# stjude-rust-labs/ngs

Measured on AMD Instinct MI355X. Metric: BAM records/sec (whole node), all qc facets, 150 bp reads, higher is better.
Workload: dtype u8/u32 integer (u64 accumulators)

## Files before the change

ngs_amd/csrc/context.cpp:

```cpp
#include <dlfcn.h>
#include <hip/hip_runtime_api.h>

#include <algorithm>
#include <atomic>
#include <cstdarg>
#include <cstdlib>
#include <cstdio>
#include <cstring>
#include <string>
#include <thread>
#include <vector>

#include "../../include/ngsq.h"
#include "../../include/ngsq_shared.h"
#include "context.h"
#include "mem_pool.h"

using namespace ngsq;

namespace ngsq {
void free_exchange_scratch(void *p);
}

static thread_local std::string g_err;
// ... 239 lines not shown
        c->n_td = round_up(c->n_cov_hist + n_bins + NGSQ_VAF_BINS, 8);
        CTX_TRY(hipMalloc((void **)&c->d_td, c->n_td * 8));
        CTX_TRY(hipMemsetAsync(c->d_td, 0, c->n_td * 8, c->stream));
        c->d_cov_hist = c->d_td;
        c->d_bin_totals = c->d_td + c->n_cov_hist;
        c->d_vaf = c->d_td + c->n_cov_hist + n_bins;
        CTX_TRY(hipMalloc((void **)&c->d_touched, 16));
        CTX_TRY(hipMemcpyAsync(c->d_touched, c->h_touched, 16, hipMemcpyHostToDevice, c->stream));
        st.touched = c->d_touched;
    }
    c->stream_cov = c->cfg.sorted_input && nd;
    if (c->stream_cov) {
        const uint64_t nr4 = round_up(nr ? nr : 1, 4);
        CTX_TRY(hipMalloc((void **)&c->d_stream_u32, (7 * nr4 + 4) * 4));
        CTX_TRY(hipMalloc((void **)&c->d_last_key, 8));
        CTX_TRY(hipMalloc((void **)&c->d_chunk_flags, round_up(c->n_chunks ? c->n_chunks : 1, 16)));
        st.end_acc = c->d_stream_u32;
        st.batch_span = c->d_stream_u32 + 7 * nr4;
        CovStreamArgs &sa = c->csa;
        sa.prev_end = c->d_stream_u32 + nr4;
        sa.plan_a = c->d_stream_u32 + 2 * nr4;
        sa.plan_z = c->d_stream_u32 + 3 * nr4;
        sa.plan_h = c->d_stream_u32 + 4 * nr4;
        sa.plan_t = c->d_stream_u32 + 5 * nr4;
        sa.guard_until = c->d_stream_u32 + 6 * nr4;
        sa.last_key = c->d_last_key;
        sa.chunk_flags = c->d_chunk_flags;
        sa.hist = c->d_cov_hist;
        sa.bin_totals = c->d_bin_totals;
        sa.bin_off = c->d_bin_off;
        sa.bin_size = c->cfg.bin_size;
        sa.cov_cap = c->cfg.cov_cap;
        sa.head_guard = c->cfg.cov_head_guard;
        CTX_TRY(hipMemsetAsync(c->d_stream_u32, 0, (7 * nr4 + 4) * 4, c->stream));
        CTX_TRY(hipMemsetAsync(sa.plan_a, 0xFF, nr4 * 4, c->stream));
        CTX_TRY(hipMemsetAsync(c->d_last_key, 0, 8, c->stream));
        CTX_TRY(hipMemsetAsync(c->d_chunk_flags, 0, c->n_chunks ? c->n_chunks : 1, c->stream));
    }
    if (ne) {
        CTX_TRY(hipMalloc((void **)&st.edits, ne * 4 + 64));
        CTX_TRY(hipMemsetAsync(st.edits, 0, ne * 4 + 64, c->stream));
        uint8_t *bases = nullptr;
        CTX_TRY(hipMalloc((void **)&bases, 2 * nbases + 256));
        CTX_TRY(hipMemsetAsync(bases, 0, 2 * nbases + 256, c->stream));
        st.ref_bases = bases;
        st.ref_bases_odd = bases + nbases;
        c->d_ref_bases = bases;
        uint8_t *codes = nullptr;
        unsigned long long *d_bad = nullptr, h_bad = 0;
        CTX_TRY(hipMalloc((void **)&codes, (deferred ? 0 : max_len) + 64));
        CTX_TRY(hipMalloc((void **)&d_bad, 8));
        CTX_TRY(hipMemsetAsync(d_bad, 0, 8, c->stream));
        uint64_t n_carry = 0;
        c->edits_carry_off.assign(nr, 0);
        std::vector<uint32_t> have(2 * (size_t)nr, 0);
        bool lens_differ = false;
        for (uint32_t r = 0; r < nr; r++) {
            if (bases_off[r] == NO_DEPTH) continue;
            const uint64_t L = c->ref_len[r];
            const uint64_t have_r = cfg->ref_bases_len && !deferred ? std::min<uint64_t>(cfg->ref_bases_len[r], L) : L;
            have[nr + r] = (uint32_t)have_r;
            have[r] = cfg->ref_bases_len && !deferred ? cfg->ref_bases_len[r] : (uint32_t)L;
            lens_differ = lens_differ || have[r] != L;
            if (!deferred && have_r) {
                CTX_TRY(hipMemcpyAsync(codes, cfg->ref_bases[r], have_r, hipMemcpyHostToDevice, c->stream));
                CTX_TRY(launch_pack_reference(c->li, codes, have_r, bases + bases_off[r], bases + nbases + bases_off[r], L / 2 + 1, d_bad, c->stream));
// ... 4 lines not shown
        }
        if (lens_differ) {
            CTX_TRY(hipMalloc((void **)&c->d_edits_len, have.size() * 4));
            CTX_TRY(hipMemcpy(c->d_edits_len, have.data(), have.size() * 4, hipMemcpyHostToDevice));
            st.ref_edits_len = c->d_edits_len;
            st.ref_fast_len = c->d_edits_len + nr;
        }
        CTX_TRY(hipStreamSynchronize(c->stream));
        CTX_TRY(hipMemcpy(&h_bad, d_bad, 8, hipMemcpyDeviceToHost));
        (void)hipFree(codes);
        (void)hipFree(d_bad);
        if (h_bad) {
            ngsq_destroy(c);
            return fail(nullptr, NGSQ_ERR_INVALID_ARGUMENT, "ngsq_config.ref_bases: every byte must be a 4-bit BAM base code (0..15)");
        }
        CTX_TRY(hipMalloc((void **)&c->d_edits_carry, (n_carry + 4) * 4));
        c->edits_conv_lo.assign(nr, 0);
        c->edits_conv_hi.assign(nr, 0);
    }
    c->h_vaf.assign(NGSQ_VAF_BINS, 0);
    for (int k = 0; k < K_COUNT; k++) c->timing[k] = {KERNEL_NAMES[k], 0, 0.0, 0};
    CTX_TRY(hipStreamSynchronize(c->stream));
#undef CTX_TRY
    *out = c;
    return NGSQ_OK;
}

void ngsq_destroy(ngsq_ctx *c) {
    if (!c) return;
    (void)hipSetDevice(c->device);
    ngsq::reference_abandon(c);
    (void)ngsq::pool_trim();
    if (c->stream) (void)hipStreamSynchronize(c->stream);
    (void)hipFree(c->d_ft_idx);
    (void)hipFree(c->d_ft_starts);
    (void)hipFree(c->d_ft_stops);
    (void)hipFree(c->d_ft_primary);
    for (const ngsq_ctx::DeferredFeatures &d : c->ft_deferred) (void)hipFree(d.buf);
    for (auto &p : c->pending) {
        (void)hipEventDestroy(p.a);
        (void)hipEventDestroy(p.b);
    }
    for (auto &ev : c->event_pool) (void)hipEventDestroy(ev);
    for (int k = 0; k < 2; k++) {
        if (c->stage[k].buf) (void)hipFree(c->stage[k].buf);
        if (c->stage[k].done) (void)hipEventDestroy(c->stage[k].done);
    }
    if (c->copy_done) (void)hipEventDestroy(c->copy_done);
    (void)hipFree(c->st.counters);
    (void)hipFree(c->st.depth);
    (void)hipFree(c->st.edits);
    (void)hipFree(c->d_ref_bases);
    (void)hipFree(c->d_edits_len);
    (void)hipFree(c->d_bad_off);
    (void)hipFree(c->d_bad_pos);
    (void)hipFree(c->d_edits_carry);
    (void)hipFree(c->d_edits_td);
    (void)hipFree(c->d_edits_defer);
    (void)hipFree(c->d_ref_len);
    (void)hipFree(c->d_depth_off);
    (void)hipFree(c->d_edits_off);
    (void)hipFree(c->d_bases_off);
    (void)hipFree(c->d_first_chunk);
    (void)hipFree(c->d_bin_off);
    (void)hipFree(c->d_td);
    (void)hipFree(c->d_touched);
// ... 124 lines not shown
        off += round_up(n ? n : 1, 256);
        return p;
    }
};

struct ColumnSizes {
    uint64_t seq_bytes, qual_bytes, cigar_ops;
};

static int column_sizes(ngsq_ctx *c, const ngsq_batch *b, ColumnSizes *cs) {
    const uint64_t n = b->n_records;
    const bool host = b->location == NGSQ_MEM_HOST;
    cs->seq_bytes = b->seq_bytes;
    cs->qual_bytes = b->qual_bytes;
    cs->cigar_ops = b->cigar_ops;
    if (!b->seq) cs->seq_bytes = 0;
    else if (!b->seq_off) cs->seq_bytes = n * b->seq_stride;
    else if (host) cs->seq_bytes = b->seq_off[n];
    if (!b->qual) cs->qual_bytes = 0;
    else if (!b->qual_off) cs->qual_bytes = n * b->qual_stride;
    else if (host) cs->qual_bytes = b->qual_off[n];
    if (!b->cigar) cs->cigar_ops = 0;
    else if (!b->cigar_off) cs->cigar_ops = n * b->cigar_stride;
    else if (host) cs->cigar_ops = b->cigar_off[n];
    (void)c;
    return NGSQ_OK;
}

static int launch_all(ngsq_ctx *c, const DeviceBatch &db, const ColumnSizes &cs, uint32_t pass_mask) {
    const uint32_t facets = c->cfg.facets;
    const uint64_t n = db.n;
    const uint32_t rec_f = (pass_mask & NGSQ_PASS_RECORD) ? (facets & NGSQ_FACETS_RECORD_BASED) : 0;
    const uint32_t seq_f = (pass_mask & NGSQ_PASS_SEQUENCE) ? (facets & NGSQ_FACETS_SEQUENCE_BASED) : 0;
    if ((rec_f & (NGSQ_FACET_GENERAL | NGSQ_FACET_TEMPLATE_LENGTH)) || (seq_f & NGSQ_FACET_COVERAGE)) {
        const bool walk = (rec_f & NGSQ_FACET_GENERAL) || (seq_f & NGSQ_FACET_COVERAGE);
        const bool cov = (seq_f & NGSQ_FACET_COVERAGE) != 0;
        if (cov && c->stream_cov) {
            const uint64_t need = round_up(n, 1024) + 1024;
            if (c->cov_end_cap < need) {
                HIP_TRY(c, hipStreamSynchronize(c->stream));
                (void)hipFree(c->d_cov_end);
                c->d_cov_end = nullptr;
                c->cov_end_cap = 0;
                HIP_TRY(c, hipMalloc((void **)&c->d_cov_end, need * 4));
                c->cov_end_cap = need;
                c->st.cov_end = c->d_cov_end;
            }
            uint32_t *const spans = c->d_stream_u32 + 7 * round_up(c->st.n_refs ? c->st.n_refs : 1, 4);
            c->st.batch_span = spans + (c->span_turn & 1);
            c->csa.span_next = spans + ((c->span_turn & 1) ^ 1);
            c->span_turn += 1;
        }
        {
            Bracket br(c, K_FIELDS, n * 25 + (walk ? cs.cigar_ops * 4 : 0));
            HIP_TRY(c, launch_fields(c->li, c->st, db, rec_f, cov ? (c->stream_cov ? 2 : 1) : 0, c->stream));
        }
        if (cov && c->stream_cov) {
            Bracket br(c, K_COV_STREAM, n * 8);
            HIP_TRY(c, launch_cov_stream(c->li, c->st, db, c->csa, c->stream));
        }
    }
    const bool gc_in_edits = (rec_f & NGSQ_FACET_GC_CONTENT) && (seq_f & NGSQ_FACET_EDITS) && edits_can_take_gc(c->st, db);
    if ((rec_f & NGSQ_FACET_GC_CONTENT) && !gc_in_edits) {
        Bracket br(c, K_GC, n * 6 + cs.seq_bytes);
        HIP_TRY(c, launch_gc(c->li, c->st, db, cs.seq_bytes, c->stream));
    }
    if (rec_f & NGSQ_FACET_QUALITY_SCORE) {
        Bracket br(c, K_QUAL, cs.qual_bytes);
        HIP_TRY(c, launch_qual(c->li, c->st, db, c->stream));
    }
    if (rec_f & NGSQ_FACET_FEATURES) {
        if (!c->have_features) {
            ngsq_ctx::DeferredFeatures d{nullptr, 0, n};
            const uint64_t n16 = round_up(n, 16);
            HIP_TRY(c, ngsq::pool_device_alloc((void **)&d.buf, n16 * 16 + 256, &d.bytes));
            c->ft_deferred.push_back(d);
            Bracket br(c, K_FEATURES, n * 12 + cs.cigar_ops * 4);
            HIP_TRY(c, launch_features_defer(c->li, db, reinterpret_cast<uint16_t *>(d.buf + n16 * 12), reinterpret_cast<int32_t *>(d.buf),
                                             reinterpret_cast<int32_t *>(d.buf + n16 * 4), reinterpret_cast<uint16_t *>(d.buf + n16 * 14),
                                             reinterpret_cast<uint32_t *>(d.buf + n16 * 8), c->stream));
        } else {
            Bracket br(c, K_FEATURES, n * 12 + cs.cigar_ops * 4);
            HIP_TRY(c, launch_features(c->li, c->st, db, c->ft, c->stream));
        }
    }
    if (seq_f & NGSQ_FACET_EDITS) {
        if (c->ref_deferred && !c->ref_ready) {
            if (!c->ref_loader) return fail(c, NGSQ_ERR_STATE, "ngsq_config.ref_bases_deferred is set but ngsq_reference_load was not called");
            const int rc = reference_join(c);
            if (rc != NGSQ_OK) return rc;
        }
        Bracket br(c, K_EDITS, n * 16 + cs.cigar_ops * 4 + cs.seq_bytes);
        const uint64_t words = (n + 63) / 64 + 16;
        if (c->edits_defer_cap < words) {
            HIP_TRY(c, hipStreamSynchronize(c->stream));
            (void)hipFree(c->d_edits_defer);
            c->d_edits_defer = nullptr;
            c->edits_defer_cap = 0;
// ... 740 lines not shown
```

ngs_amd/csrc/context.h:

```cpp
#pragma once

#include <hip/hip_runtime_api.h>

#include <string>
#include <vector>

#include "../../include/ngsq.h"
#include "kernels.h"

struct ngsq_ctx;

namespace ngsq {

enum KernelId { K_FIELDS = 0, K_GC, K_QUAL, K_EDITS, K_COV_SCAN, K_EDITS_VAF, K_H2D, K_FEATURES, K_COV_STREAM, K_INFLATE, K_INFLATE_CRC,
                K_REC_INDEX, K_REC_COLUMNS, K_COUNT };

struct PendingTime {
    int id;
    hipEvent_t a, b;
};

struct KernelTimer {
    ngsq_ctx *c;
    int id;
// ... 39 lines not shown
    uint32_t *d_edits_carry = nullptr;
    uint8_t *d_edits_td = nullptr;
    size_t edits_td_cap = 0;
    std::vector<uint8_t> h_edits_td;
    unsigned long long *d_edits_defer = nullptr;
    uint64_t edits_defer_cap = 0;
    std::vector<uint64_t> edits_carry_off, edits_conv_lo, edits_conv_hi;
    uint32_t *d_first_chunk = nullptr;
    uint64_t *d_bin_off = nullptr;
    uint64_t n_diff = 0, n_chunks = 0;
    unsigned long long *d_td = nullptr;
    uint64_t n_td = 0;
    unsigned long long *d_touched = nullptr;
    unsigned long long h_touched[2] = {~0ull, 0};
    uint64_t scan_lo = 0, scan_hi = 0;
    uint32_t scan_carry = 0;
    const uint32_t *scan_words = nullptr;
    uint64_t scan_front = 0;
    uint32_t vaf_part = 0, vaf_parts = 1;
    void *xchg_scratch = nullptr;
    bool scan_partial = false, torn_down = false;
    unsigned long long *d_cov_hist = nullptr, *d_bin_totals = nullptr, *d_vaf = nullptr;
    std::vector<unsigned long long> h_counters, h_cov_hist, h_bin_totals, h_vaf;
    bool finalized = false;
    bool edits_uploaded = false;
    unsigned long long *pin_results = nullptr, *pin_results_dev = nullptr;
    uint64_t pin_words = 0;
    bool stream_cov = false;
    uint32_t *d_cov_end = nullptr;
    uint64_t cov_end_cap = 0;
    uint32_t *d_stream_u32 = nullptr;
    unsigned long long *d_last_key = nullptr;
    uint32_t span_turn = 0;
    uint8_t *d_chunk_flags = nullptr;
    ngsq::CovStreamArgs csa{};
    ngsq::FeatureTables ft{};
    uint32_t *d_ft_idx = nullptr, *d_ft_starts = nullptr, *d_ft_stops = nullptr;
    uint8_t *d_ft_primary = nullptr;
    bool have_features = false;
    struct DeferredFeatures {
        uint8_t *buf;
        size_t bytes;
        uint64_t n;
    };
    std::vector<DeferredFeatures> ft_deferred;
    ngsq::Staging stage[2];
    int stage_next = 0;
    ngsq_kernel_time timing[ngsq::K_COUNT]{};
    std::vector<ngsq::PendingTime> pending;
    std::vector<hipEvent_t> event_pool;
    std::string err;
};
```

ngs_amd/csrc/cov_stream.hip:

```cpp
#include <hip/hip_runtime.h>

#include <type_traits>

#include "kernels.h"

namespace ngsq {

typedef unsigned long long u64;

constexpr uint32_t ST_THREADS = 256;
constexpr uint32_t ST_WAVES = ST_THREADS / 64;
constexpr uint32_t ST_W = 1024;
constexpr uint32_t ST_LIST = 232;
constexpr uint32_t ST_HOT_BINS = 64, ST_HOT_REP = 4, ST_HOT = ST_HOT_BINS * ST_HOT_REP;

__device__ __forceinline__ u64 st_key(int32_t rf, int32_t ps) {
    return rf < 0 ? 0xFFFFFFFF00000000ull : ((u64)(uint32_t)rf << 32) | (uint32_t)(ps + 1);
}
__device__ __forceinline__ bool st_valid(const DeviceState &st, int32_t rf, int32_t ps) {
    return rf >= 0 && (uint32_t)rf < st.n_refs && ps >= 0 && st.ref_depth_off[rf] != NO_DEPTH;
}

__global__ __launch_bounds__(256) void k_cov_plan_tiles(DeviceState st, DeviceBatch b, CovStreamArgs a) {
    NGSQ_FOREGROUND_WAVE();
// ... 3 lines not shown
        const u64 k0 = st_key(b.ref_id[0], b.pos[0]);
        if (k0 < *a.last_key) atomicAdd(&st.counters[C_COV_UNSORTED], 1ull);
        *a.last_key = st_key(b.ref_id[b.n - 1], b.pos[b.n - 1]);
    }
    const uint32_t lane = threadIdx.x & 63u;
    auto first_of = [&](int64_t u, int32_t &r, int32_t &p) {
        const bool ok = u >= 0 && (uint64_t)u < n_wt;
        r = ok ? b.ref_id[(uint64_t)u * CS_TILE] : -1;
        p = ok ? b.pos[(uint64_t)u * CS_TILE] : -1;
    };
    int32_t rf[4], ps[4];
    first_of((int64_t)t, rf[1], ps[1]);
    rf[0] = __shfl_up(rf[1], 1, 64), ps[0] = __shfl_up(ps[1], 1, 64);
    rf[2] = __shfl_down(rf[1], 1, 64), ps[2] = __shfl_down(ps[1], 1, 64);
    rf[3] = __shfl_down(rf[1], 2, 64), ps[3] = __shfl_down(ps[1], 2, 64);
    if (lane == 0) first_of((int64_t)t - 1, rf[0], ps[0]);
    if (lane == 63) first_of((int64_t)t + 1, rf[2], ps[2]);
    if (lane >= 62) first_of((int64_t)t + 2, rf[3], ps[3]);
    if (t >= n_wt) return;
    auto streamable = [&](int k) {
        return st_valid(st, rf[k], ps[k]) && rf[k + 1] == rf[k] && ps[k + 1] >= 0;
    };
    if (!streamable(1)) return;
    const bool prev_same = streamable(0) && rf[0] == rf[1];
    const bool next_same = streamable(2) && rf[2] == rf[1];
    if (!prev_same) atomicMin(&a.plan_a[rf[1]], (uint32_t)ps[1] + 1);
    if (!next_same) atomicMax(&a.plan_z[rf[1]], (uint32_t)ps[2] + 1);
}

__global__ __launch_bounds__(256) void k_cov_plan_refs(DeviceState st, CovStreamArgs a) {
    NGSQ_FOREGROUND_WAVE();
    const uint32_t r = blockIdx.x * blockDim.x + threadIdx.x;
    if (r == 0 && a.span_next) *a.span_next = 0;
    if (r >= st.n_refs) return;
    const uint32_t pa = a.plan_a[r], pz = a.plan_z[r], prev = a.prev_end[r];
    const uint32_t acc = st.end_acc[r];
    uint32_t guard = a.guard_until[r];
    if (a.head_guard && guard == 0 && (pa != CS_NONE || acc != 0)) {
        const uint64_t g = (uint64_t)(pa != CS_NONE ? pa : acc) + a.head_guard;
        guard = g > 0xFFFFFFFEull ? 0xFFFFFFFEu : (uint32_t)g;
        a.guard_until[r] = guard;
    }
    uint32_t H = CS_NONE, T = CS_NONE;
    if (pa != CS_NONE && pz > pa) {
        uint64_t base = pa > prev + 1 ? pa : (uint64_t)prev + 1;
        if (guard > base) base = guard;
        const uint64_t h = (base + COV_CHUNK - 1) / COV_CHUNK * COV_CHUNK;
        const uint64_t lim = pz < (uint64_t)st.ref_len[r] + 1 ? pz : (uint64_t)st.ref_len[r] + 1;
        const uint64_t tt = lim / COV_CHUNK * COV_CHUNK;
        if (h < tt) {
            H = (uint32_t)h;
            T = (uint32_t)tt;
        }
    }
    a.plan_h[r] = H;
    a.plan_t[r] = T;
    a.prev_end[r] = acc > prev ? acc : prev;
    a.plan_a[r] = CS_NONE;
    a.plan_z[r] = 0;
}

__device__ __forceinline__ uint32_t st_wave_scan(uint32_t v) {
    v += (uint32_t)__builtin_amdgcn_update_dpp(0, (int)v, 0x111, 0xF, 0xF, false);
    v += (uint32_t)__builtin_amdgcn_update_dpp(0, (int)v, 0x112, 0xF, 0xF, false);
    v += (uint32_t)__builtin_amdgcn_update_dpp(0, (int)v, 0x114, 0xF, 0xF, false);
    v += (uint32_t)__builtin_amdgcn_update_dpp(0, (int)v, 0x118, 0xF, 0xF, false);
    v += (uint32_t)__builtin_amdgcn_update_dpp(0, (int)v, 0x142, 0xA, 0xF, false);
    v += (uint32_t)__builtin_amdgcn_update_dpp(0, (int)v, 0x143, 0xC, 0xF, false);
    return v;
}
__device__ __forceinline__ uint32_t st_wave_max(uint32_t v) {
#pragma unroll
    for (int o = 32; o > 0; o >>= 1) v = max(v, (uint32_t)__shfl_xor(v, o, 64));
    return v;
}

__host__ __device__ inline uint32_t st_hist_words(uint32_t cov_cap) { return ((cov_cap + 2 + 1) / 2 + 3) & ~3u; }

constexpr uint32_t ST_PER_LANE = 8;
constexpr uint32_t ST_PASS = 64 * ST_PER_LANE;
static_assert(ST_W % ST_PASS == 0, "whole passes");

struct StTileIn {
    int4 p;
    uint4 c;
    int32_t rf_t, ps_t, rf_n, ps_n;
};

constexpr uint32_t ST_MIN_BLOCKS = 4;
__global__ __launch_bounds__(ST_THREADS, ST_MIN_BLOCKS) void k_cov_stream(DeviceState st, DeviceBatch b, CovStreamArgs a) {
    NGSQ_FOREGROUND_WAVE();
    extern __shared__ __attribute__((aligned(16))) uint32_t s_dyn[];
    const uint32_t nb = a.cov_cap + 2;
    const uint32_t tid = threadIdx.x, lane = tid & 63;
    const uint32_t wave = (uint32_t)__builtin_amdgcn_readfirstlane((int)(tid >> 6));
    const uint32_t hw = st_hist_words(a.cov_cap);
    uint32_t *const win = s_dyn + wave * (ST_W + hw + ST_HOT + ST_LIST);
    uint32_t *const hist = win + ST_W;
    uint32_t *const hot = hist + hw;
    uint32_t *const lst = hot + ST_HOT;
    for (uint32_t i = lane; i < ST_W + hw + ST_HOT + ST_LIST; i += 64) win[i] = 0;
    __builtin_amdgcn_fence(__ATOMIC_ACQ_REL, "wavefront");
    __builtin_amdgcn_wave_barrier();

    const uint64_t n_wt = (b.n + CS_TILE - 1) / CS_TILE;
    const uint64_t n_full = b.n / CS_TILE;
    const uint64_t n_units = (uint64_t)gridDim.x * ST_WAVES, unit = (uint64_t)blockIdx.x * ST_WAVES + wave;
    const uint64_t per = (n_wt + n_units - 1) / n_units;
    const uint64_t t_begin = per * unit < n_wt ? per * unit : n_wt;
    const uint64_t t_end = t_begin + per < n_wt ? t_begin + per : n_wt;
    const uint32_t maxspan = *st.batch_span;

    uint32_t hot_base = 0;
    int32_t hist_ref = -1;
    uint32_t since_flush = 0;
    u64 zero_run = 0;
    uint32_t lane_zero = 0;
    u64 *bins = a.bin_totals;
    u64 lane_bin = 0;
    uint32_t bin_q = 0, bin_p0 = 1, bin_p1 = 0;
    u64 t_lo = ~0ull, t_hi = 0;
    bool lst_valid = false;
    uint64_t lst_tile = 0;
    int32_t lst_ref = -1;
    uint32_t lst_lo = 0, lst_n = 0;
    int32_t plan_ref = -1;
    uint32_t pH = CS_NONE, pT = CS_NONE, pL = 0;
    uint64_t pOff = 0;

    auto flush_bin = [&]() {
        u64 v = lane_bin;
#pragma unroll
        for (int o = 32; o > 0; o >>= 1) v += __shfl_xor(v, o, 64);
        if (lane == 0 && v) atomicAdd(&bins[bin_q], v);
        lane_bin = 0;
    };
    auto flush_hot = [&]() {
        static_assert((ST_HOT_REP == 4 || ST_HOT_REP == 8) && ST_HOT_BINS <= 64, "one or two uint4 per lane");
        uint4 *const cell = reinterpret_cast<uint4 *>(hot) + (lane < ST_HOT_BINS ? lane : 0u) * (ST_HOT_REP / 4);
        uint32_t t = 0;
        if (lane < ST_HOT_BINS) {
#pragma unroll
            for (uint32_t q = 0; q < ST_HOT_REP / 4; q++) {
// ... 303 lines not shown
                    __builtin_amdgcn_wave_barrier();
                }
            }
        }

        if (from_list) {
            for (uint32_t c = 0; c < lst_n; c += 64) {
                const uint32_t ee = c + lane < lst_n ? lst[c + lane] : 0u;
                const u64 km = __ballot(ee > hi);
                if (ee > hi) lst[new_n + __builtin_amdgcn_mbcnt_hi((uint32_t)(km >> 32), __builtin_amdgcn_mbcnt_lo((uint32_t)km, 0))] = ee;
                new_n += (uint32_t)__popcll(km);
            }
        }
#pragma unroll
        for (uint32_t j = 0; j < 4; j++) {
            const u64 km = __ballot(e[j] > hi);
            const uint32_t kn = (uint32_t)__popcll(km);
            if (new_ok && new_n + kn <= ST_LIST) {
                if (e[j] > hi) lst[new_n + __builtin_amdgcn_mbcnt_hi((uint32_t)(km >> 32), __builtin_amdgcn_mbcnt_lo((uint32_t)km, 0))] = e[j];
                new_n += kn;
            } else {
                new_ok = false;
            }
        }
        lst_valid = new_ok;
        lst_n = new_n;
        lst_tile = t + 1;
        lst_ref = rf_t;
        lst_lo = hi;
        __builtin_amdgcn_fence(__ATOMIC_ACQ_REL, "wavefront");
        __builtin_amdgcn_wave_barrier();
    };

    uint64_t t = t_begin;
    const uint64_t t_full_end = t_end < n_full ? t_end : n_full;
    if (t < t_full_end) {
        StTileIn cur = load_full(t);
        while (t < t_full_end) {
            const uint64_t tn = t + 1;
            const StTileIn nxt = load_full(tn < n_full ? tn : t);
            process(cur, t);
            cur = nxt;
            t = tn;
        }
    }
    if (n_full < n_wt && t_begin <= n_full && n_full < t_end) {
        const uint64_t base = n_full * CS_TILE, r0 = base + (uint64_t)lane * 4;
        int32_t p[4];
        uint32_t c[4];
#pragma unroll
        for (uint32_t j = 0; j < 4; j++) {
            const bool ok = r0 + j < b.n;
            p[j] = ok ? b.pos[r0 + j] : -1;
            c[j] = ok ? st.cov_end[r0 + j] : 0u;
        }
        StTileIn in;
        in.p = make_int4(p[0], p[1], p[2], p[3]);
        in.c = make_uint4(c[0], c[1], c[2], c[3]);
        in.rf_t = in.rf_n = b.ref_id[base];
        in.ps_t = in.ps_n = b.pos[base];
        process(in, n_full);
    }
    flush_hist();
    flush_bin();
#pragma unroll
    for (int o = 32; o > 0; o >>= 1) {
        const u64 l2 = __shfl_xor(t_lo, o, 64), h2 = __shfl_xor(t_hi, o, 64);
        t_lo = l2 < t_lo ? l2 : t_lo;
        t_hi = h2 > t_hi ? h2 : t_hi;
    }
    if (lane == 0 && t_hi > 0) {
        atomicMin(&st.touched[0], t_lo);
        atomicMax(&st.touched[1], t_hi);
    }
}

hipError_t launch_cov_stream(const LaunchInfo &li, const DeviceState &st, const DeviceBatch &b, const CovStreamArgs &a,
                             hipStream_t s) {
    if (!b.n) return hipSuccess;
    const uint64_t n_wt = (b.n + CS_TILE - 1) / CS_TILE;
    hipLaunchKernelGGL(k_cov_plan_tiles, dim3((uint32_t)((n_wt + 255) / 256)), dim3(256), 0, s, st, b, a);
    hipLaunchKernelGGL(k_cov_plan_refs, dim3((st.n_refs + 255) / 256), dim3(256), 0, s, st, a);
    const size_t lds = (size_t)ST_WAVES * (ST_W + st_hist_words(a.cov_cap) + ST_HOT + ST_LIST) * sizeof(uint32_t);
    static bool attr = false;
    if (!attr) {
        hipError_t e = hipFuncSetAttribute(reinterpret_cast<const void *>(k_cov_stream),
                                           hipFuncAttributeMaxDynamicSharedMemorySize, 160 * 1024 - 64);
        if (e != hipSuccess) return e;
        attr = true;
    }
    uint64_t g = (n_wt + ST_WAVES - 1) / ST_WAVES;
    const uint64_t per_cu = (160 * 1024 - 1024) / lds;
    const uint64_t cap = (uint64_t)li.n_cu * (per_cu < 1 ? 1 : per_cu > 6 ? 6 : per_cu);
    if (g > cap) g = cap;
    hipLaunchKernelGGL(k_cov_stream, dim3((uint32_t)g), dim3(ST_THREADS), lds, s, st, b, a);
    return hipGetLastError();
}

}
```

ngs_amd/csrc/kernels.h:

```cpp
#pragma once

#include <hip/hip_runtime_api.h>
#include <stdint.h>

#include "../../include/ngsq.h"

#define NGSQ_FOREGROUND_WAVE() __builtin_amdgcn_s_setprio(3)

namespace ngsq {

enum : uint32_t {
    C_GENERAL = 0,
    C_CIGAR1 = 16,
    C_CIGAR2 = 25,
    C_TLEN_PROCESSED = 34,
    C_TLEN_IGNORED = 35,
    C_GC_GC = 36,
    C_GC_AT = 37,
    C_GC_OTHER = 38,
    C_GC_PROCESSED = 39,
    C_GC_IGN_FLAGS = 40,
    C_GC_IGN_SHORT = 41,
    C_COV_NONSENSICAL = 42,
    C_ERR = 43,
    E_MISSING_REF = 0,
    E_BAD_QUAL = 1,
    E_READ_TOO_LONG = 2,
    E_EDITS_BAD_REF = 3,
    E_EDITS_SHORT = 4,
    E_EDITS_NOT_CONSUMED = 5,
    E_EDITS_TOO_MANY = 6,
    E_BAD_CIGAR = 7,
    C_FEAT = 51,
    F_UTR5 = 0,
    F_UTR3 = 1,
    F_CDS = 2,
    F_INTERGENIC = 3,
    F_EXONIC = 4,
    F_INTRONIC = 5,
    F_PROCESSED = 6,
// ... 57 lines not shown
    const uint64_t *record_id;
    uint64_t qual_bytes;
};

#if defined(__HIPCC__)
__device__ __forceinline__ uint32_t batch_n_ops(const DeviceBatch &b, uint64_t i) {
    uint32_t n = b.n_cigar[i];
    if (n == 0xFFFFu && b.cigar_off) n = (uint32_t)(b.cigar_off[i + 1] - b.cigar_off[i]);
    return n;
}
#endif

struct LaunchInfo {
    int n_cu;
};

hipError_t launch_fields(const LaunchInfo &li, const DeviceState &st, const DeviceBatch &b,
                         uint32_t rec_facets, int coverage, hipStream_t s);

constexpr uint32_t CS_TILE = 256;
constexpr uint32_t CS_NONE = 0xFFFFFFFFu;
struct CovStreamArgs {
    uint32_t *plan_a, *plan_z;
    uint32_t *plan_h, *plan_t;
    uint32_t *prev_end;
    uint32_t *guard_until;
    unsigned long long *last_key;
    uint8_t *chunk_flags;
    unsigned long long *hist;
    unsigned long long *bin_totals;
    const uint64_t *bin_off;
    uint32_t bin_size, cov_cap, head_guard;
    uint32_t *span_next;
};
hipError_t launch_cov_stream(const LaunchInfo &li, const DeviceState &st, const DeviceBatch &b, const CovStreamArgs &a,
                             hipStream_t s);
hipError_t launch_gc(const LaunchInfo &li, const DeviceState &st, const DeviceBatch &b,
                     uint64_t seq_bytes, hipStream_t s);
hipError_t launch_qual(const LaunchInfo &li, const DeviceState &st, const DeviceBatch &b,
                       hipStream_t s);
bool qual_window_supported(const DeviceState &st, const DeviceBatch &b);
hipError_t launch_qual_window(const LaunchInfo &li, const DeviceState &st, const DeviceBatch &b, hipStream_t s);
struct FeatureTables {
    const uint32_t *idx;
    const uint32_t *starts;
    const uint32_t *stops;
    const uint8_t *primary;
    uint32_t n_refs;
    uint32_t role_name[5];
    unsigned long long *scratch;
};
constexpr uint32_t FT_SLOTS = 32;
hipError_t launch_features_defer(const LaunchInfo &li, const DeviceBatch &b, uint16_t *flag, int32_t *ref, int32_t *pos, uint16_t *ncig, uint32_t *cig,
                                 hipStream_t s);
hipError_t launch_features(const LaunchInfo &li, const DeviceState &st, const DeviceBatch &b, const FeatureTables &ft,
                           hipStream_t s);
bool qual_ragged_supported(const DeviceState &st, const DeviceBatch &b);
hipError_t launch_qual_ragged(const LaunchInfo &li, const DeviceState &st, const DeviceBatch &b, hipStream_t s);
bool edits_can_take_gc(const DeviceState &st, const DeviceBatch &b);
hipError_t launch_edits(const LaunchInfo &li, const DeviceState &st, const DeviceBatch &b, unsigned long long *defer_bits, bool with_gc,
                        hipStream_t s);

constexpr uint32_t COV_CHUNK = 4096;
constexpr uint32_t COV_SUPER = 256;
struct CovScanArgs {
    uint32_t *depth;
    uint64_t n_chunks;
    uint64_t c_begin, c_end;
    uint32_t carry_in;
    const uint32_t *carry_words;
    uint64_t carry_mask;
// ... 75 lines not shown
```

ngs_amd/csrc/kernels.hip:

```cpp
#include <hip/hip_runtime.h>

#include "../../include/ngsq_shared.h"
#include "kernels.h"

namespace ngsq {

typedef unsigned long long u64;

__device__ __forceinline__ uint32_t wave_sum(uint32_t v) {
#pragma unroll
    for (int o = 32; o > 0; o >>= 1) v += __shfl_down(v, o, 64);
    return v;
}
__device__ __forceinline__ u64 wave_sum64(u64 v) {
#pragma unroll
    for (int o = 32; o > 0; o >>= 1) v += __shfl_down(v, o, 64);
    return v;
}

template <int N>
__device__ __forceinline__ void block_flush(const uint32_t (&v)[N], u64 *s_acc, u64 *dst,
                                            const uint32_t (&idx)[N]) {
    const int lane = threadIdx.x & 63;
#pragma unroll
    for (int k = 0; k < N; k++) {
        uint32_t r = wave_sum(v[k]);
        if (lane == 0 && r) atomicAdd(&s_acc[k], (u64)r);
    }
    __syncthreads();
    for (int k = threadIdx.x; k < N; k += blockDim.x) {
        u64 r = s_acc[k];
        if (r) atomicAdd(&dst[idx[k]], r);
    }
}

__device__ __forceinline__ void block_slice(uint64_t n, uint64_t &lo, uint64_t &hi) {
    const uint64_t per = (n + gridDim.x - 1) / gridDim.x;
    lo = per * blockIdx.x;
    hi = lo + per;
    if (lo > n) lo = n;
    if (hi > n) hi = n;
}

__device__ __forceinline__ void gc_dword(uint32_t x, uint32_t mask, uint32_t &gc, uint32_t &at) {
    const uint32_t y = x >> 1, z = x >> 2, u = x >> 3;
    gc += __popc((y ^ z) & ~(x | u) & mask);
    at += __popc((x ^ u) & ~(y | z) & mask);
}

template <bool OFFS, bool RID>
__global__ __launch_bounds__(256) void k_gc(DeviceState st, DeviceBatch b, uint64_t seq_bytes) {
    NGSQ_FOREGROUND_WAVE();
    __shared__ uint32_t s_hist[NGSQ_GC_BINS];
    __shared__ u64 s_acc[6];
    if (threadIdx.x < NGSQ_GC_BINS) s_hist[threadIdx.x] = 0;
    if (threadIdx.x < 6) s_acc[threadIdx.x] = 0;
    __syncthreads();
    uint32_t c[6] = {0, 0, 0, 0, 0, 0};
    constexpr uint32_t M = 0x11111111u;

    uint64_t lo, hi;
    block_slice(b.n, lo, hi);
    struct Info {
        uint32_t f, l;
        uint64_t row, rid;
    };
    auto fetch = [&](uint64_t j) -> Info {
        Info r;
        r.f = b.flag[j];
        r.l = b.l_seq[j];
        r.row = OFFS ? b.seq_off[j] : j * (uint64_t)b.seq_stride;
        r.rid = RID ? b.record_id[j] : b.first_record_index + j;
        return r;
    };
    const uint64_t step = blockDim.x, i0 = lo + threadIdx.x;
    Info nx{0, 0, 0, 0};
    if (i0 < hi) nx = fetch(i0);
    for (uint64_t i = i0; i < hi; i += step) {
        const Info r = nx;
        nx = fetch(i + step < hi ? i + step : i);
        if (r.f & 0x500u) {
            c[4] += 1;
            continue;
        }
        if (r.l < NGSQ_GC_WINDOW) {
// ... 72 lines not shown
            for (uint32_t cyc = st.max_read_len + lane; cyc < nq; cyc += 64)
                over |= (!fixed_row || q[cyc] != 0xFFu);
            if (__any(over) && lane == 0) c[1] += 1;
            nq = st.max_read_len;
        }
        for (uint32_t cyc = lane; cyc < nq; cyc += 64) {
            const uint32_t v = q[cyc];
            if (fixed_row && v == 0xFFu) continue;
            if (v > NGSQ_MAX_SCORE) {
                c[0] += 1;
            } else if (cyc < lds_rows) {
                atomicAdd(&s_q[cyc * QUAL_BINS + v], 1u);
            } else {
                atomicAdd(&st.counters[st.off_qual + (uint64_t)cyc * QUAL_BINS + v], 1ull);
            }
        }
    }
    __syncthreads();
    for (uint32_t i = threadIdx.x; i < nbins; i += blockDim.x) {
        uint32_t v = s_q[i];
        if (v) atomicAdd(&st.counters[st.off_qual + i], (u64)v);
    }
    const uint32_t idx[2] = {C_ERR + E_BAD_QUAL, C_ERR + E_READ_TOO_LONG};
    block_flush<2>(c, s_acc, st.counters, idx);
}

static inline uint32_t grid_for(uint64_t n, uint32_t per_block, uint32_t max_blocks) {
    uint64_t g = (n + per_block - 1) / per_block;
    if (g < 1) g = 1;
    if (g > max_blocks) g = max_blocks;
    return (uint32_t)g;
}

hipError_t launch_gc(const LaunchInfo &li, const DeviceState &st, const DeviceBatch &b, uint64_t seq_bytes,
                     hipStream_t s) {
    if (!b.n) return hipSuccess;
    const uint32_t grid = grid_for(b.n, 256 * 4, li.n_cu * 8);
    if (b.seq_off && b.record_id) hipLaunchKernelGGL((k_gc<true, true>), dim3(grid), dim3(256), 0, s, st, b, seq_bytes);
    else if (b.seq_off) hipLaunchKernelGGL((k_gc<true, false>), dim3(grid), dim3(256), 0, s, st, b, seq_bytes);
    else if (b.record_id) hipLaunchKernelGGL((k_gc<false, true>), dim3(grid), dim3(256), 0, s, st, b, seq_bytes);
    else hipLaunchKernelGGL((k_gc<false, false>), dim3(grid), dim3(256), 0, s, st, b, seq_bytes);
    return hipGetLastError();
}

hipError_t launch_qual(const LaunchInfo &li, const DeviceState &st, const DeviceBatch &b, hipStream_t s) {
    if (!b.n) return hipSuccess;
    if (qual_window_supported(st, b)) return launch_qual_window(li, st, b, s);
    if (qual_ragged_supported(st, b)) return launch_qual_ragged(li, st, b, s);
    uint32_t rows = b.qual_off ? st.max_read_len : b.qual_stride;
    if (rows > st.max_read_len) rows = st.max_read_len;
    if (rows > QUAL_LDS_MAX_ROWS) rows = QUAL_LDS_MAX_ROWS;
    if (rows < 1) rows = 1;
    const size_t lds = (size_t)rows * QUAL_BINS * sizeof(uint32_t);
    static bool attr_set = false;
    if (!attr_set) {
        hipError_t e = hipFuncSetAttribute(reinterpret_cast<const void *>(k_qual_general),
                                           hipFuncAttributeMaxDynamicSharedMemorySize,
                                           QUAL_LDS_MAX_ROWS * QUAL_BINS * sizeof(uint32_t));
        if (e != hipSuccess) return e;
        attr_set = true;
    }
    const uint32_t per_cu = lds <= 72 * 1024 ? 2 : 1;
    const uint32_t grid = grid_for(b.n, 1024, li.n_cu * per_cu);
    hipLaunchKernelGGL(k_qual_general, dim3(grid), dim3(1024), lds, s, st, b, rows);
    return hipGetLastError();
}

__global__ __launch_bounds__(256) void k_state_spans(StateSpans a) {
    const uint64_t q = (uint64_t)blockIdx.x * blockDim.x + threadIdx.x;
    uint32_t k = 0;
    uint64_t base = 0;
#pragma unroll 1
    for (; k < a.n; k++) {
        const uint64_t quads = (a.span[k].n_words + 3) / 4;
// ... 32 lines not shown
```

Measured before the change: 18.47 billion.

## Co-run streamed coverage on a side stream beside GC content kernel

Splits the coverage planning launch out and, when both coverage and GC facets are active, forks the streamed coverage kernel onto a side stream so it runs concurrently with the GC kernel, joining via events. The co-run coverage kernel uses an atomic run counter for dynamic work distribution in fixed-length tile runs, and both kernels launch with fewer blocks per CU so they can share the device; GC waves get a lower priority. Intent is to fill idle CU capacity left by each kernel alone, at the cost of extra event/stream overhead, contention between the two kernels, and reduced occupancy for each.

```diff
diff --git a/ngs_amd/csrc/context.cpp b/ngs_amd/csrc/context.cpp
--- a/ngs_amd/csrc/context.cpp
+++ b/ngs_amd/csrc/context.cpp
@@ -295,6 +295,12 @@
         sa.bin_size = c->cfg.bin_size;
         sa.cov_cap = c->cfg.cov_cap;
         sa.head_guard = c->cfg.cov_head_guard;
+        sa.run_next = c->d_stream_u32 + 7 * nr4 + 2;
+        int prio = 0;
+        CTX_TRY(hipStreamGetPriority(c->stream, &prio));
+        CTX_TRY(hipStreamCreateWithPriority(&c->side_stream, hipStreamNonBlocking, prio));
+        CTX_TRY(hipEventCreateWithFlags(&c->side_fork, hipEventDisableTiming));
+        CTX_TRY(hipEventCreateWithFlags(&c->side_join, hipEventDisableTiming));
         CTX_TRY(hipMemsetAsync(c->d_stream_u32, 0, (7 * nr4 + 4) * 4, c->stream));
         CTX_TRY(hipMemsetAsync(sa.plan_a, 0xFF, nr4 * 4, c->stream));
         CTX_TRY(hipMemsetAsync(c->d_last_key, 0, 8, c->stream));
@@ -365,6 +371,12 @@
     ngsq::reference_abandon(c);
     (void)ngsq::pool_trim();
     if (c->stream) (void)hipStreamSynchronize(c->stream);
+    if (c->side_stream) {
+        (void)hipStreamSynchronize(c->side_stream);
+        (void)hipStreamDestroy(c->side_stream);
+    }
+    if (c->side_fork) (void)hipEventDestroy(c->side_fork);
+    if (c->side_join) (void)hipEventDestroy(c->side_join);
     (void)hipFree(c->d_ft_idx);
     (void)hipFree(c->d_ft_starts);
     (void)hipFree(c->d_ft_stops);
@@ -555,6 +567,8 @@
     const uint64_t n = db.n;
     const uint32_t rec_f = (pass_mask & NGSQ_PASS_RECORD) ? (facets & NGSQ_FACETS_RECORD_BASED) : 0;
     const uint32_t seq_f = (pass_mask & NGSQ_PASS_SEQUENCE) ? (facets & NGSQ_FACETS_SEQUENCE_BASED) : 0;
+    const bool gc_in_edits = (rec_f & NGSQ_FACET_GC_CONTENT) && (seq_f & NGSQ_FACET_EDITS) && edits_can_take_gc(c->st, db);
+    const bool corun = (seq_f & NGSQ_FACET_COVERAGE) && c->stream_cov && (rec_f & NGSQ_FACET_GC_CONTENT) && !gc_in_edits && n;
     if ((rec_f & (NGSQ_FACET_GENERAL | NGSQ_FACET_TEMPLATE_LENGTH)) || (seq_f & NGSQ_FACET_COVERAGE)) {
         const bool walk = (rec_f & NGSQ_FACET_GENERAL) || (seq_f & NGSQ_FACET_COVERAGE);
         const bool cov = (seq_f & NGSQ_FACET_COVERAGE) != 0;
@@ -579,14 +593,34 @@
             HIP_TRY(c, launch_fields(c->li, c->st, db, rec_f, cov ? (c->stream_cov ? 2 : 1) : 0, c->stream));
         }
         if (cov && c->stream_cov) {
-            Bracket br(c, K_COV_STREAM, n * 8);
-            HIP_TRY(c, launch_cov_stream(c->li, c->st, db, c->csa, c->stream));
-        }
-    }
-    const bool gc_in_edits = (rec_f & NGSQ_FACET_GC_CONTENT) && (seq_f & NGSQ_FACET_EDITS) && edits_can_take_gc(c->st, db);
-    if ((rec_f & NGSQ_FACET_GC_CONTENT) && !gc_in_edits) {
+            HIP_TRY(c, launch_cov_plan(c->st, db, c->csa, c->stream));
+            if (corun) {
+                HIP_TRY(c, hipEventRecord(c->side_fork, c->stream));
+                HIP_TRY(c, hipStreamWaitEvent(c->side_stream, c->side_fork, 0));
+                hipError_t e;
+                {
+                    Bracket br(c, K_COV_STREAM, n * 8, c->side_stream);
+                    e = launch_cov_stream(c->li, c->st, db, c->csa, true, c->side_stream);
+                }
+                if (e == hipSuccess) {
+                    Bracket br(c, K_GC, n * 6 + cs.seq_bytes);
+                    e = launch_gc(c->li, c->st, db, cs.seq_bytes, true, c->stream);
+                }
+                if (e == hipSuccess) e = hipEventRecord(c->side_join, c->side_stream);
+                if (e == hipSuccess) e = hipStreamWaitEvent(c->stream, c->side_join, 0);
+                if (e != hipSuccess) {
+                    (void)hipStreamSynchronize(c->side_stream);
+                    return fail(c, NGSQ_ERR_DEVICE, "streamed Coverage beside GC Content failed: %s", hipGetErrorString(e));
+                }
+            } else {
+                Bracket br(c, K_COV_STREAM, n * 8);
+                HIP_TRY(c, launch_cov_stream(c->li, c->st, db, c->csa, false, c->stream));
+            }
+        }
+    }
+    if ((rec_f & NGSQ_FACET_GC_CONTENT) && !gc_in_edits && !corun) {
         Bracket br(c, K_GC, n * 6 + cs.seq_bytes);
-        HIP_TRY(c, launch_gc(c->li, c->st, db, cs.seq_bytes, c->stream));
+        HIP_TRY(c, launch_gc(c->li, c->st, db, cs.seq_bytes, false, c->stream));
     }
     if (rec_f & NGSQ_FACET_QUALITY_SCORE) {
         Bracket br(c, K_QUAL, cs.qual_bytes);
diff --git a/ngs_amd/csrc/context.h b/ngs_amd/csrc/context.h
--- a/ngs_amd/csrc/context.h
+++ b/ngs_amd/csrc/context.h
@@ -95,6 +95,8 @@
     uint32_t *d_stream_u32 = nullptr;
     unsigned long long *d_last_key = nullptr;
     uint32_t span_turn = 0;
+    hipStream_t side_stream = nullptr;
+    hipEvent_t side_fork = nullptr, side_join = nullptr;
     uint8_t *d_chunk_flags = nullptr;
     ngsq::CovStreamArgs csa{};
     ngsq::FeatureTables ft{};
diff --git a/ngs_amd/csrc/cov_stream.hip b/ngs_amd/csrc/cov_stream.hip
--- a/ngs_amd/csrc/cov_stream.hip
+++ b/ngs_amd/csrc/cov_stream.hip
@@ -59,6 +59,7 @@
     NGSQ_FOREGROUND_WAVE();
     const uint32_t r = blockIdx.x * blockDim.x + threadIdx.x;
     if (r == 0 && a.span_next) *a.span_next = 0;
+    if (r == 0) *a.run_next = 0;
     if (r >= st.n_refs) return;
     const uint32_t pa = a.plan_a[r], pz = a.plan_z[r], prev = a.prev_end[r];
     const uint32_t acc = st.end_acc[r];
@@ -114,8 +115,8 @@
     int32_t rf_t, ps_t, rf_n, ps_n;
 };
 
-constexpr uint32_t ST_MIN_BLOCKS = 4;
-__global__ __launch_bounds__(ST_THREADS, ST_MIN_BLOCKS) void k_cov_stream(DeviceState st, DeviceBatch b, CovStreamArgs a) {
+template <bool CORUN>
+__device__ __forceinline__ void cov_stream_body(const DeviceState &st, const DeviceBatch &b, const CovStreamArgs &a, uint32_t run_len) {
     NGSQ_FOREGROUND_WAVE();
     extern __shared__ __attribute__((aligned(16))) uint32_t s_dyn[];
     const uint32_t nb = a.cov_cap + 2;
@@ -132,10 +133,6 @@
 
     const uint64_t n_wt = (b.n + CS_TILE - 1) / CS_TILE;
     const uint64_t n_full = b.n / CS_TILE;
-    const uint64_t n_units = (uint64_t)gridDim.x * ST_WAVES, unit = (uint64_t)blockIdx.x * ST_WAVES + wave;
-    const uint64_t per = (n_wt + n_units - 1) / n_units;
-    const uint64_t t_begin = per * unit < n_wt ? per * unit : n_wt;
-    const uint64_t t_end = t_begin + per < n_wt ? t_begin + per : n_wt;
     const uint32_t maxspan = *st.batch_span;
 
     uint32_t hot_base = 0;
@@ -505,34 +502,49 @@
         __builtin_amdgcn_wave_barrier();
     };
 
-    uint64_t t = t_begin;
-    const uint64_t t_full_end = t_end < n_full ? t_end : n_full;
-    if (t < t_full_end) {
-        StTileIn cur = load_full(t);
-        while (t < t_full_end) {
-            const uint64_t tn = t + 1;
-            const StTileIn nxt = load_full(tn < n_full ? tn : t);
-            process(cur, t);
-            cur = nxt;
-            t = tn;
-        }
-    }
-    if (n_full < n_wt && t_begin <= n_full && n_full < t_end) {
-        const uint64_t base = n_full * CS_TILE, r0 = base + (uint64_t)lane * 4;
-        int32_t p[4];
-        uint32_t c[4];
-#pragma unroll
-        for (uint32_t j = 0; j < 4; j++) {
-            const bool ok = r0 + j < b.n;
-            p[j] = ok ? b.pos[r0 + j] : -1;
-            c[j] = ok ? st.cov_end[r0 + j] : 0u;
-        }
-        StTileIn in;
-        in.p = make_int4(p[0], p[1], p[2], p[3]);
-        in.c = make_uint4(c[0], c[1], c[2], c[3]);
-        in.rf_t = in.rf_n = b.ref_id[base];
-        in.ps_t = in.ps_n = b.pos[base];
-        process(in, n_full);
+    auto tiles_from = [&](uint64_t t_begin) {
+        const uint64_t t_end = t_begin + run_len < n_wt ? t_begin + run_len : n_wt;
+        uint64_t t = t_begin;
+        const uint64_t t_full_end = t_end < n_full ? t_end : n_full;
+        if (t < t_full_end) {
+            StTileIn cur = load_full(t);
+            while (t < t_full_end) {
+                const uint64_t tn = t + 1;
+                const StTileIn nxt = load_full(tn < n_full ? tn : t);
+                process(cur, t);
+                cur = nxt;
+                t = tn;
+            }
+        }
+        if (n_full < n_wt && t_begin <= n_full && n_full < t_end) {
+            const uint64_t base = n_full * CS_TILE, r0 = base + (uint64_t)lane * 4;
+            int32_t p[4];
+            uint32_t c[4];
+#pragma unroll
+            for (uint32_t j = 0; j < 4; j++) {
+                const bool ok = r0 + j < b.n;
+                p[j] = ok ? b.pos[r0 + j] : -1;
+                c[j] = ok ? st.cov_end[r0 + j] : 0u;
+            }
+            StTileIn in;
+            in.p = make_int4(p[0], p[1], p[2], p[3]);
+            in.c = make_uint4(c[0], c[1], c[2], c[3]);
+            in.rf_t = in.rf_n = b.ref_id[base];
+            in.ps_t = in.ps_n = b.pos[base];
+            process(in, n_full);
+        }
+    };
+    if constexpr (CORUN) {
+        for (;;) {
+            uint32_t run = 0;
+            if (lane == 0) run = atomicAdd(a.run_next, 1u);
+            const uint64_t t_begin = (uint64_t)(uint32_t)__builtin_amdgcn_readfirstlane((int)run) * run_len;
+            if (t_begin >= n_wt) break;
+            tiles_from(t_begin);
+        }
+    } else {
+        const uint64_t t_begin = ((uint64_t)blockIdx.x * ST_WAVES + wave) * run_len;
+        if (t_begin < n_wt) tiles_from(t_begin);
     }
     flush_hist();
     flush_bin();
@@ -548,25 +560,46 @@
     }
 }
 
-hipError_t launch_cov_stream(const LaunchInfo &li, const DeviceState &st, const DeviceBatch &b, const CovStreamArgs &a,
-                             hipStream_t s) {
+__global__ __launch_bounds__(ST_THREADS, 4) void k_cov_stream(DeviceState st, DeviceBatch b, CovStreamArgs a, uint32_t run_len) {
+    cov_stream_body<false>(st, b, a, run_len);
+}
+__global__ __launch_bounds__(ST_THREADS, 3) void k_cov_stream_corun(DeviceState st, DeviceBatch b, CovStreamArgs a, uint32_t run_len) {
+    cov_stream_body<true>(st, b, a, run_len);
+}
+
+hipError_t launch_cov_plan(const DeviceState &st, const DeviceBatch &b, const CovStreamArgs &a, hipStream_t s) {
     if (!b.n) return hipSuccess;
     const uint64_t n_wt = (b.n + CS_TILE - 1) / CS_TILE;
     hipLaunchKernelGGL(k_cov_plan_tiles, dim3((uint32_t)((n_wt + 255) / 256)), dim3(256), 0, s, st, b, a);
     hipLaunchKernelGGL(k_cov_plan_refs, dim3((st.n_refs + 255) / 256), dim3(256), 0, s, st, a);
+    return hipGetLastError();
+}
+
+constexpr uint32_t CS_CORUN_BLOCKS = 3;
+hipError_t launch_cov_stream(const LaunchInfo &li, const DeviceState &st, const DeviceBatch &b, const CovStreamArgs &a,
+                             bool corun, hipStream_t s) {
+    if (!b.n) return hipSuccess;
+    const uint64_t n_wt = (b.n + CS_TILE - 1) / CS_TILE;
     const size_t lds = (size_t)ST_WAVES * (ST_W + st_hist_words(a.cov_cap) + ST_HOT + ST_LIST) * sizeof(uint32_t);
     static bool attr = false;
     if (!attr) {
-        hipError_t e = hipFuncSetAttribute(reinterpret_cast<const void *>(k_cov_stream),
-                                           hipFuncAttributeMaxDynamicSharedMemorySize, 160 * 1024 - 64);
-        if (e != hipSuccess) return e;
+        for (const void *k : {reinterpret_cast<const void *>(k_cov_stream), reinterpret_cast<const void *>(k_cov_stream_corun)}) {
+            hipError_t e = hipFuncSetAttribute(k, hipFuncAttributeMaxDynamicSharedMemorySize, 160 * 1024 - 64);
+            if (e != hipSuccess) return e;
+        }
         attr = true;
     }
+    const uint64_t per_cu = (160 * 1024 - 1024) / lds;
+    const uint64_t fit = per_cu < 1 ? 1 : per_cu > 6 ? 6 : per_cu;
+    const uint64_t cap = (uint64_t)li.n_cu * (corun && fit > CS_CORUN_BLOCKS ? CS_CORUN_BLOCKS : fit);
     uint64_t g = (n_wt + ST_WAVES - 1) / ST_WAVES;
-    const uint64_t per_cu = (160 * 1024 - 1024) / lds;
-    const uint64_t cap = (uint64_t)li.n_cu * (per_cu < 1 ? 1 : per_cu > 6 ? 6 : per_cu);
     if (g > cap) g = cap;
-    hipLaunchKernelGGL(k_cov_stream, dim3((uint32_t)g), dim3(ST_THREADS), lds, s, st, b, a);
+    const uint64_t share = (n_wt + g * ST_WAVES - 1) / (g * ST_WAVES);
+    const uint32_t run_len = (uint32_t)(corun && share > CS_RUN ? CS_RUN : share);
+    const uint64_t n_runs = (n_wt + run_len - 1) / run_len;
+    if (g > (n_runs + ST_WAVES - 1) / ST_WAVES) g = (n_runs + ST_WAVES - 1) / ST_WAVES;
+    if (corun) hipLaunchKernelGGL(k_cov_stream_corun, dim3((uint32_t)g), dim3(ST_THREADS), lds, s, st, b, a, run_len);
+    else hipLaunchKernelGGL(k_cov_stream, dim3((uint32_t)g), dim3(ST_THREADS), lds, s, st, b, a, run_len);
     return hipGetLastError();
 }
 
diff --git a/ngs_amd/csrc/kernels.h b/ngs_amd/csrc/kernels.h
--- a/ngs_amd/csrc/kernels.h
+++ b/ngs_amd/csrc/kernels.h
@@ -6,6 +6,7 @@
 #include "../../include/ngsq.h"
 
 #define NGSQ_FOREGROUND_WAVE() __builtin_amdgcn_s_setprio(3)
+#define NGSQ_BESIDE_FOREGROUND_WAVE() __builtin_amdgcn_s_setprio(2)
 
 namespace ngsq {
 
@@ -129,11 +130,14 @@
     const uint64_t *bin_off;
     uint32_t bin_size, cov_cap, head_guard;
     uint32_t *span_next;
-};
+    uint32_t *run_next;
+};
+constexpr uint32_t CS_RUN = 48;
+hipError_t launch_cov_plan(const DeviceState &st, const DeviceBatch &b, const CovStreamArgs &a, hipStream_t s);
 hipError_t launch_cov_stream(const LaunchInfo &li, const DeviceState &st, const DeviceBatch &b, const CovStreamArgs &a,
-                             hipStream_t s);
+                             bool corun, hipStream_t s);
 hipError_t launch_gc(const LaunchInfo &li, const DeviceState &st, const DeviceBatch &b,
-                     uint64_t seq_bytes, hipStream_t s);
+                     uint64_t seq_bytes, bool corun, hipStream_t s);
 hipError_t launch_qual(const LaunchInfo &li, const DeviceState &st, const DeviceBatch &b,
                        hipStream_t s);
 bool qual_window_supported(const DeviceState &st, const DeviceBatch &b);
diff --git a/ngs_amd/csrc/kernels.hip b/ngs_amd/csrc/kernels.hip
--- a/ngs_amd/csrc/kernels.hip
+++ b/ngs_amd/csrc/kernels.hip
@@ -49,8 +49,9 @@
 }
 
 template <bool OFFS, bool RID>
-__global__ __launch_bounds__(256) void k_gc(DeviceState st, DeviceBatch b, uint64_t seq_bytes) {
-    NGSQ_FOREGROUND_WAVE();
+__global__ __launch_bounds__(256) void k_gc(DeviceState st, DeviceBatch b, uint64_t seq_bytes, uint32_t corun) {
+    if (corun) NGSQ_BESIDE_FOREGROUND_WAVE();
+    else NGSQ_FOREGROUND_WAVE();
     __shared__ uint32_t s_hist[NGSQ_GC_BINS];
     __shared__ u64 s_acc[6];
     if (threadIdx.x < NGSQ_GC_BINS) s_hist[threadIdx.x] = 0;
@@ -189,14 +190,16 @@
     return (uint32_t)g;
 }
 
-hipError_t launch_gc(const LaunchInfo &li, const DeviceState &st, const DeviceBatch &b, uint64_t seq_bytes,
+constexpr uint32_t GC_BLOCKS = 8, GC_CORUN_BLOCKS = 4, GC_CORUN_BLOCKS_WIDE = 3;
+hipError_t launch_gc(const LaunchInfo &li, const DeviceState &st, const DeviceBatch &b, uint64_t seq_bytes, bool corun,
                      hipStream_t s) {
     if (!b.n) return hipSuccess;
-    const uint32_t grid = grid_for(b.n, 256 * 4, li.n_cu * 8);
-    if (b.seq_off && b.record_id) hipLaunchKernelGGL((k_gc<true, true>), dim3(grid), dim3(256), 0, s, st, b, seq_bytes);
-    else if (b.seq_off) hipLaunchKernelGGL((k_gc<true, false>), dim3(grid), dim3(256), 0, s, st, b, seq_bytes);
-    else if (b.record_id) hipLaunchKernelGGL((k_gc<false, true>), dim3(grid), dim3(256), 0, s, st, b, seq_bytes);
-    else hipLaunchKernelGGL((k_gc<false, false>), dim3(grid), dim3(256), 0, s, st, b, seq_bytes);
+    const uint32_t per_cu = !corun ? GC_BLOCKS : b.seq_off || b.record_id ? GC_CORUN_BLOCKS_WIDE : GC_CORUN_BLOCKS;
+    const uint32_t grid = grid_for(b.n, 256 * 4, li.n_cu * per_cu);
+    if (b.seq_off && b.record_id) hipLaunchKernelGGL((k_gc<true, true>), dim3(grid), dim3(256), 0, s, st, b, seq_bytes, corun ? 1u : 0u);
+    else if (b.seq_off) hipLaunchKernelGGL((k_gc<true, false>), dim3(grid), dim3(256), 0, s, st, b, seq_bytes, corun ? 1u : 0u);
+    else if (b.record_id) hipLaunchKernelGGL((k_gc<false, true>), dim3(grid), dim3(256), 0, s, st, b, seq_bytes, corun ? 1u : 0u);
+    else hipLaunchKernelGGL((k_gc<false, false>), dim3(grid), dim3(256), 0, s, st, b, seq_bytes, corun ? 1u : 0u);
     return hipGetLastError();
 }
 
```

After: 19.74 billion, median of 6. +6.9%, better.
